# okieraised/rs-face-detection-tflite

Hardware: AMD Instinct MI355X
Metric: faces/sec at batch=256 (256x256 back-camera) per GPU (higher is better)
Workload: dtype f32

## Files before the change

rs-face-detection-tflite_amd/csrc/strip_kernels.hip:

```cpp
#include <hip/hip_runtime.h>

#include <algorithm>
#include <cstdint>
#include <cstdio>
#include <cstdlib>
#include <type_traits>

#include "kernels.hpp"
#include "launch.hpp"

namespace mi {

namespace {

typedef float sf32x16 __attribute__((ext_vector_type(16)));
typedef float v2f __attribute__((ext_vector_type(2)));
typedef float v4f __attribute__((ext_vector_type(4)));
typedef unsigned v2u __attribute__((ext_vector_type(2)));
typedef float __attribute__((address_space(4))) cfloat;

struct StripArgs {
    const float* in;
    float* out;
    const float* consts;
// ... 529 lines not shown
        if (has_skip) {
#pragma unroll
            for (int q = 0; q < CQ; q++) {
                oacc[2 * q] = v2f{mx[q].x, mx[q].y} + v2f{bp[4 * q], bp[4 * q + 1]};
                oacc[2 * q + 1] = v2f{mx[q].z, mx[q].w} + v2f{bp[4 * q + 2], bp[4 * q + 3]};
            }
        } else {
#pragma unroll
            for (int q = 0; q < CQ; q++) {
                oacc[2 * q] = v2f{bp[4 * q], bp[4 * q + 1]};
                oacc[2 * q + 1] = v2f{bp[4 * q + 2], bp[4 * q + 3]};
            }
        }
#pragma unroll
        for (int o = 0; o < 2 * CQ; o++) asm volatile("" : "+v"(oacc[o]));
    }
    load_first(0);
    load_x(0, xbuf[0]);
#pragma unroll
    for (int st = 0; st < 2 * CQ; st++) {
        const int q = st >> 1, h = st & 1;
        __builtin_amdgcn_s_waitcnt(0xC07F);
        if (MODE == 2) load_second(st);
        __builtin_amdgcn_sched_barrier(0);
        const float4 (&x)[3] = xbuf[q & 1];
        if (h == 0) {
            float4 m = make_float4(fmaxf(x[0].x, x[1].x), fmaxf(x[0].y, x[1].y), fmaxf(x[0].z, x[1].z), fmaxf(x[0].w, x[1].w));
            if (MODE == 0) m = make_float4(fmaxf(m.x, mx[q].x), fmaxf(m.y, mx[q].y), fmaxf(m.z, mx[q].z), fmaxf(m.w, mx[q].w));
            mx[q] = m;
        }
        v2f t[3];
#pragma unroll
        for (int kx = 0; kx < 3; kx++) t[kx] = h == 0 ? v2f{x[kx].x, x[kx].y} : v2f{x[kx].z, x[kx].w};
        auto wv = [&](int tap) { return v2f{wd[2 * tap], wd[2 * tap + 1]}; };
        v2f pch = acc[q][h], n;
        if (MODE == 0) {
            n = pch;
#pragma unroll
            for (int kx = 0; kx < 3; kx++) n = pkfma(t[kx], wv(3 + kx), n);
        } else {
            n = t[0] * wv(0);
#pragma unroll
            for (int kx = 0; kx < 3; kx++) {
                if (MODE == 2) pch = pkfma(t[kx], wv(6 + kx), pch);
                if (kx) n = pkfma(t[kx], wv(kx), n);
            }
        }
        acc[q][h] = n;
        asm volatile("" : "+v"(acc[q][h]));
        if constexpr (MODE == 2) {
#pragma unroll
            for (int o = 0; o < 2 * CQ; o++) oacc[o] = pkfma(v2f{pch.x, pch.x}, v2f{wp0[2 * o], wp0[2 * o + 1]}, oacc[o]);
            asm volatile("" : "+v"(pch));
        }
        __builtin_amdgcn_sched_barrier(0);
        __builtin_amdgcn_s_waitcnt(0xC07F);
        if (st + 1 < 2 * CQ) {
            load_first(st + 1);
            if (h == 1) load_x(q + 1, xbuf[(q + 1) & 1]);
        }
        __builtin_amdgcn_sched_barrier(0);
        if constexpr (MODE == 2) {
#pragma unroll
            for (int o = 0; o < 2 * CQ; o++) {
                oacc[o] = pkfma(v2f{pch.y, pch.y}, v2f{wp1[2 * o], wp1[2 * o + 1]}, oacc[o]);
                asm volatile("" : "+v"(oacc[o]));
            }
        }
        __builtin_amdgcn_sched_barrier(0);
    }
}

template <int CQ, int NH, int MODE, int PS>
__device__ __forceinline__ void strip_row_s2m(const float* me2, const cfloat* cst, int hf, bool has_skip, v2f (&acc)[CQ][2], float4 (&mx)[CQ],
                                              v4f (&oacc)[CQ], const float (&wa)[SK<CQ>::NA]) {
    constexpr int C = 4 * CQ, Co = NH * C;
    constexpr int ST2 = (32 + 2 * Co + 15) / 16 * 16, OFF_BIAS2 = (C / 2) * ST2;
    float wd[2][18];
    float4 xbuf[2][3];
    auto load_taps = [&](int st) {
        const cfloat* p = cst;
        asm volatile("" : "+s"(p));
#pragma unroll
        for (int i = 0; i < 18; i++) wd[st & 1][i] = p[st * ST2 + i];
    };
    auto load_x = [&](int q, float4 (&x)[3]) {
#pragma unroll
        for (int kx = 0; kx < 3; kx++) x[kx] = sld4(me2 + kx * PS + 4 * q);
    };
    if constexpr (MODE == 2) {
        const cfloat* bp = cst + OFF_BIAS2 + hf * C;
        asm volatile("" : "+s"(bp));
        if (has_skip) {
#pragma unroll
            for (int q = 0; q < CQ; q++) oacc[q] = v4f{mx[q].x, mx[q].y, mx[q].z, mx[q].w} + v4f{bp[4 * q], bp[4 * q + 1], bp[4 * q + 2], bp[4 * q + 3]};
        } else {
#pragma unroll
            for (int q = 0; q < CQ; q++) oacc[q] = v4f{bp[4 * q], bp[4 * q + 1], bp[4 * q + 2], bp[4 * q + 3]};
        }
#pragma unroll
        for (int q = 0; q < CQ; q++) asm volatile("" : "+v"(oacc[q]));
    }
    load_taps(0);
    load_x(0, xbuf[0]);
#pragma unroll
    for (int st = 0; st < 2 * CQ; st++) {
        const int q = st >> 1, h = st & 1;
        __builtin_amdgcn_s_waitcnt(0xC07F);
        if (st + 1 < 2 * CQ) {
            load_taps(st + 1);
            if (h == 1) load_x(q + 1, xbuf[(q + 1) & 1]);
        }
        __builtin_amdgcn_sched_barrier(0);
        const float4 (&x)[3] = xbuf[q & 1];
        if (h == 0) {
            float4 m = make_float4(fmaxf(x[0].x, x[1].x), fmaxf(x[0].y, x[1].y), fmaxf(x[0].z, x[1].z), fmaxf(x[0].w, x[1].w));
            if (MODE == 0) m = make_float4(fmaxf(m.x, mx[q].x), fmaxf(m.y, mx[q].y), fmaxf(m.z, mx[q].z), fmaxf(m.w, mx[q].w));
            mx[q] = m;
        }
        v2f t[3];
#pragma unroll
        for (int kx = 0; kx < 3; kx++) t[kx] = h == 0 ? v2f{x[kx].x, x[kx].y} : v2f{x[kx].z, x[kx].w};
        const float (&w)[18] = wd[st & 1];
        auto wv = [&](int tap) { return v2f{w[2 * tap], w[2 * tap + 1]}; };
        v2f pch = acc[q][h], n;
        if (MODE == 0) {
            n = pch;
#pragma unroll
            for (int kx = 0; kx < 3; kx++) n = pkfma(t[kx], wv(3 + kx), n);
        } else {
            n = t[0] * wv(0);
#pragma unroll
            for (int kx = 0; kx < 3; kx++) {
                if (MODE == 2) pch = pkfma(t[kx], wv(6 + kx), pch);
                if (kx) n = pkfma(t[kx], wv(kx), n);
            }
        }
        acc[q][h] = n;
        asm volatile("" : "+v"(acc[q][h]));
        if constexpr (MODE == 2) {
            asm volatile("" : "+v"(pch));
            __builtin_amdgcn_sched_barrier(0);
#pragma unroll
            for (int e = 0; e < 2; e++) {
                const float bv = e ? pch.y : pch.x;
#pragma unroll
                for (int tq = 0; tq < CQ; tq++) {
                    const int nn = (2 * st + e) * CQ + tq;
                    oacc[tq] = mfma4_bcast(wa[nn >> 4], bv, oacc[tq], nn & 15);
                }
            }
        }
        __builtin_amdgcn_sched_barrier(0);
    }
}

template <int CQ, bool RELU>
__global__ __launch_bounds__(256, CQ <= 6 ? 3 : 2) void strip_kernel(StripArgs a) {
    using K = SK<CQ>;
    constexpr int C = K::C, NL = K::NL, BUF_F = K::BUF_F;
    extern __shared__ __attribute__((aligned(16))) float lds[];
    const int lane = threadIdx.x & 63;
    const int wave = __builtin_amdgcn_readfirstlane(threadIdx.x >> 6);
    float* wbase = lds + wave * K::WAVE_F;
    int gw = blockIdx.x * 4 + wave;
    const int band = gw % a.bands;
    gw /= a.bands;
    const int strip = gw % a.strips, b = gw / a.strips;
    if (b >= a.B) return;
    const int x0 = strip * 64;
    const int y0 = band * a.band_rows, y1 = min(y0 + a.band_rows, a.H);
    if (y0 >= y1) return;
    const float* in = a.in + (long)b * a.in_fs;
    float* out = a.out + (long)b * a.out_fs;
    const cfloat* cst = (const cfloat*)a.consts;

    int goff[NL];
#pragma unroll
    for (int k = 0; k < NL; k++) {
        const int f = min(lane + 64 * k, K::NF - 1), px = f / CQ, qd = f - px * CQ;
        goff[k] = (min(max(x0 - 1 + px, 0), a.W - 1) * C + 4 * qd) * 4;
    }
    const int npx = min(64, a.W - x0);
    const bool full = npx == 64;
    const int zl = x0 == 0 ? 0 : -1;
    const int zr = x0 + 64 >= a.W ? npx + 1 : -1;
    const long gout = (long)x0 * C + 4 * lane;
    const unsigned lds_wave = __builtin_amdgcn_readfirstlane((unsigned)(uintptr_t)(__attribute__((address_space(3))) float*)wbase);

    auto issue_row = [&](int r, int bi) {
        const char* src = reinterpret_cast<const char*>(in + (long)min(max(r, 0), a.H - 1) * a.W * C);
        const unsigned dstb = lds_wave + (unsigned)(bi * BUF_F * 4);
        constexpr int TAIL = K::NF - 64 * (NL - 1);
#pragma unroll
        for (int k = 0; k < NL; k++) {
            if (k < NL - 1 || TAIL == 64) {
                asm volatile("s_mov_b32 m0, %0\n\ts_nop 0\n\tglobal_load_lds_dwordx4 %1, %2" ::"s"(dstb + 1024u * k), "v"(goff[k]), "s"(src) : "memory", "m0");
            } else {
                unsigned long long saved;
                asm volatile("s_mov_b64 %0, exec\n\ts_mov_b64 exec, %4\n\ts_mov_b32 m0, %1\n\ts_nop 0\n\tglobal_load_lds_dwordx4 %2, %3\n\ts_mov_b64 exec, %0"
                             : "=&s"(saved) : "s"(dstb + 1024u * k), "v"(goff[k]), "s"(src), "n"((1ull << (TAIL & 63)) - 1) : "memory", "m0");
            }
        }
    };
    const int zfix = lane < CQ ? (zl >= 0 ? zl * C + 4 * lane : -1) : (lane < 2 * CQ ? (zr >= 0 ? zr * C + 4 * (lane - CQ) : -1) : -1);
    auto fix_row = [&](int r, int bi) {
        float* buf = wbase + bi * BUF_F;
        const float4 z = make_float4(0.f, 0.f, 0.f, 0.f);
        if (r < 0 || r >= a.H) {
#pragma unroll
            for (int k = 0; k < NL; k++)
                if (64 * (k + 1) <= K::NF || lane < K::NF - 64 * k) sst4(buf + 4 * (lane + 64 * k), z);
        } else if (zfix >= 0) {
            sst4(buf + zfix, z);
        }
    };

    v2f oacc[2 * CQ];
    auto row = [&](auto emit_t, int bi, v2f (&aPN)[CQ][2], v2f (&aC)[CQ][2], const float4 (&xres)[CQ], float4 (&xcur)[CQ]) {
        strip_row<CQ, decltype(emit_t)::value>(wbase + bi * BUF_F + lane * C, cst, a.has_res != 0, aPN, aC, xres, xcur, oacc);
    };
    auto epilogue = [&](int y, int bi) {
        float* obuf = wbase + bi * BUF_F;
        float4 o[CQ];
        strip_act<CQ, RELU>(oacc, cst + K::OFF_SLOPE, a.hi, o);
#pragma unroll
        for (int q = 0; q < CQ; q++) sst4(obuf + lane * C + 4 * q, o[q]);
        wave_sync();
        float* dst = out + (long)y * a.W * C + gout;
        if (full) {
#pragma unroll
            for (int k = 0; k < CQ; k++) sst4(dst + 256 * k, sld4(obuf + 4 * lane + 256 * k));
        } else {
#pragma unroll
            for (int k = 0; k < CQ; k++) {
                const float4 o = sld4(obuf + 4 * lane + 256 * k);
                if (lane + 64 * k < npx * CQ) sst4(dst + 256 * k, o);
            }
        }
    };

    v2f acc0[CQ][2], acc1[CQ][2];
    float4 xa[CQ], xb[CQ];
#pragma unroll
    for (int q = 0; q < CQ; q++) {
        acc0[q][0] = acc0[q][1] = acc1[q][0] = acc1[q][1] = v2f{0.f, 0.f};
        xa[q] = xb[q] = make_float4(0.f, 0.f, 0.f, 0.f);
    }
#ifdef MI_STRIP_STAMPS
    unsigned long long st_acc[5] = {0, 0, 0, 0, 0}, st_prev = __builtin_amdgcn_s_memtime();
#define MI_SSTAMP(k) { __builtin_amdgcn_sched_barrier(0); unsigned long long t_ = __builtin_amdgcn_s_memtime(); __builtin_amdgcn_s_waitcnt(0xC07F); st_acc[k] += t_ - st_prev; st_prev = t_; __builtin_amdgcn_sched_barrier(0); }
#else
#define MI_SSTAMP(k)
#endif
    auto step = [&](auto emit, int r, v2f (&aPN)[CQ][2], v2f (&aC)[CQ][2], const float4 (&xprev)[CQ], float4 (&xcur)[CQ]) {
        const int bi = (r - (y0 - 1)) & 1;
        if (r + 1 <= y1) {
            if (full && r >= y0 + 2) wait_vm<NL + CQ>();
            else wait_vm<NL>();
        } else {
            wait_vm<0>();
        }
        MI_SSTAMP(0)
        fix_row(r, bi);
        wave_sync();
        MI_SSTAMP(1)
        row(emit, bi, aPN, aC, xprev, xcur);
        wave_sync();
        MI_SSTAMP(2)
        if constexpr (decltype(emit)::value) epilogue(r - 1, bi);
        wave_sync();
        if (r + 2 <= y1) issue_row(r + 2, bi);
        MI_SSTAMP(3)
    };
    issue_row(y0 - 1, 0);
    issue_row(y0, 1);
    step(std::false_type{}, y0 - 1, acc0, acc1, xb, xa);
    step(std::false_type{}, y0, acc1, acc0, xa, xb);
    for (int r = y0 + 1; r <= y1; r += 2) {
        step(std::true_type{}, r, acc0, acc1, xb, xa);
        if (r + 1 > y1) break;
        step(std::true_type{}, r + 1, acc1, acc0, xa, xb);
    }
#ifdef MI_STRIP_STAMPS
    if (a.stamps && lane == 0)
        for (int k = 0; k < 4; k++) a.stamps[((long)blockIdx.x * 4 + wave) * 8 + k] = st_acc[k];
#endif
}

constexpr int kMaxPipe = 4;
struct PipeArgs {
    const float* in;
    float* out;
    const float* consts[kMaxPipe];
    long in_fs, out_fs;
    int B, H, W;
    int strips, bands, band_rows, units;
    int rows_per_step;
    int has_res[kMaxPipe];
    float hi[kMaxPipe];
    int prio;
#ifdef MI_PIPE_STAMPS
    unsigned long long* stamps;
#endif
};

// ... 580 lines not shown
        const float4 z = make_float4(0.f, 0.f, 0.f, 0.f);
        if (e < 0 || e >= a.H) {
#pragma unroll
            for (int q = 0; q < CQ; q++) sst4(dstl + 4 * q, z);
        } else if (full) {
#pragma unroll
            for (int q = 0; q < CQ; q++) sst4(dstl + 4 * q, o[q]);
        } else {
#pragma unroll
            for (int q = 0; q < CQ; q++) sst4(dstl + 4 * q, lane >= npx ? z : o[q]);
        }
    };
    auto tail_step = [&](int t, v2f (&tacc)[CQ][2], float4 (&tmx)[CQ]) {
        if constexpr (NH2 > 0) {
            const int mt = t - 2 * S;
            if (mt < 0 || 2 * mt > a.band_rows) return;
            const int k = 2 * mt;
            constexpr int Co = NH2 * C;
            constexpr int ST2 = (32 + 2 * Co + 15) / 16 * 16, OFF_SLOPE2 = (C / 2) * ST2 + 64;
            const cfloat* cst2 = (const cfloat*)a.consts[S];
            const float* img = lds + ((S - 1) * 2) * IMG;
            const int tu = a.strips == 2 ? 0 : lane >> 5, tox = a.strips == 2 ? lane : lane & 31;
            const float* me2 = img + tu * 66 * C + (2 * tox + 1) * C;
            const bool skip = hf == 0 && a.has_res[S] != 0;
            if (mt == 0) {
                strip_row_s2<CQ, NH2, 1>(me2, cst2, hf, skip, tacc, tmx, oacc0);
            } else {
                strip_row_s2<CQ, NH2, 2>(me2, cst2, hf, skip, tacc, tmx, oacc0);
                float4 o[CQ];
                strip_act<CQ, RELU>(oacc0, cst2 + OFF_SLOPE2 + hf * C, a.hi[S], o);
                float* obuf = scratch;
#pragma unroll
                for (int q = 0; q < CQ; q++) sst4(obuf + lane * C + 4 * q, o[q]);
                wave_sync();
                const int Wo = a.W >> 1;
#pragma unroll
                for (int j = 0; j < CQ; j++) {
                    const int f = lane + 64 * j, px = f / CQ, qd = f - px * CQ;
                    const int u = a.strips == 2 ? 0 : px >> 5, ox = a.strips == 2 ? px : px & 31;
                    const int un = a.strips == 2 ? (int)blockIdx.x : 2 * (int)blockIdx.x + u;
                    const int ub = un % a.bands, bb = min(un / a.bands, a.B - 1);
                    const int uy0 = ub * a.band_rows, uy1 = min(uy0 + a.band_rows, a.H);
                    const float4 v = sld4(obuf + 4 * f);
                    if (un < a.units && uy0 + k <= uy1 && ox < Wo) {
                        const int oy = (uy0 + k - 2) >> 1;
                        sst4(a.out + (long)bb * a.out_fs + ((long)oy * Wo + ox) * Co + hf * C + 4 * qd, v);
                    }
                }
                wave_sync();
            }
            if (k + 1 < a.band_rows) strip_row_s2<CQ, NH2, 0>(me2 + IMG, cst2, hf, skip, tacc, tmx, oacc0);
        }
    };
    auto step = [&](int t, const float4 (&xin)[CQ], float4 (&xout)[CQ], v2f (&tacc)[CQ][2], float4 (&tmx)[CQ]) {
        const int m = t - 2 * role;
        const int c0 = lo_j - 1 + 2 * m;
        bool hand_over = false, store_out = false;
        float4 o0[CQ], o1[CQ];
        if (!tail && active && m >= 0 && m < P) {
            const float *me0, *me1;
            if (role == 0) {
                if (m + 1 < P) wait_vm<2 * NL>();
                else wait_vm<0>();
                fix_row(c0, (m & 1) * 2);
                fix_row(c0 + 1, (m & 1) * 2 + 1);
                wave_sync();
                me0 = scratch + ((m & 1) * 2) * BUF_F + lane * C;
                me1 = me0 + BUF_F;
            } else {
                me0 = lds + ((role - 1) * 2) * IMG + img_p + lane * C;
                me1 = me0 + IMG;
            }
            strip_row2<CQ>(me0, me1, cst, has_res, aA, aB, xin, xout, oacc0, oacc1);
            wave_sync();
            if (m >= 1) {
                strip_act<CQ, RELU>(oacc0, cst + K::OFF_SLOPE, hi, o0);
                strip_act<CQ, RELU>(oacc1, cst + K::OFF_SLOPE, hi, o1);
                if (NH2 || role < S - 1) hand_over = true;
#ifdef MI_ABL_STORE_EARLY
                else { store_row(c0 - 1, o0); store_row(c0, o1); }
#else
                else store_out = true;
#endif
            }
            if (role == 0 && m + 2 < P) {
                wave_sync();
                issue_row(c0 + 4, (m & 1) * 2);
                issue_row(c0 + 5, (m & 1) * 2 + 1);
            }
        }
        if constexpr (NH2 > 0) {
            if (tail) tail_step(t, tacc, tmx);
        }
        MI_PSTAMP(0)
        wg_barrier();
        MI_PSTAMP(1)
        if (hand_over) {
            hand_row(c0 - 1, 0, o0);
            hand_row(c0, 1, o1);
        } else if (store_out) {
            store_row(c0 - 1, o0);
            store_row(c0, o1);
        }
        MI_PSTAMP(2)
        wg_barrier();
        MI_PSTAMP(3)
    };
    const int T = NH2 ? 2 * S + a.band_rows / 2 + 1 : 2 * S - 1 + a.band_rows / 2;
    for (int t = 0; t < T; t += 2) {
        step(t, xa, xb, aA, xa);
        if (t + 1 >= T) break;
        step(t + 1, xb, xa, aA, xa);
    }
#ifdef MI_PIPE_STAMPS
    if (a.stamps && lane == 0) {
        unsigned long long* d = a.stamps + ((size_t)blockIdx.x * 8 + w) * 8;
        for (int k = 0; k < 4; k++) d[k] = ps_acc[k];
        d[4] = T;
    }
#endif
#undef MI_PSTAMP
}

template <int CQ, int KB, bool RELU, int NH2>
__global__ __launch_bounds__(NH2 ? 128 * (KB - 1) + 64 * NH2 : 128 * KB, 2) void strip_pipe2m_kernel(PipeArgs a) {
    using K = SK<CQ>;
    constexpr int C = K::C, NL = K::NL, BUF_F = K::BUF_F;
    constexpr int S = NH2 ? KB - 1 : KB;
    constexpr int NT = 128 * S + 64 * NH2;
    constexpr int PXS = C + 4;
    constexpr int IMG = 132 * PXS;
    constexpr int RING_F = (KB - 1) * 2 * IMG;
    extern __shared__ __attribute__((aligned(16))) float lds[];
    const int lane = threadIdx.x & 63;
    const int w = __builtin_amdgcn_readfirstlane(threadIdx.x >> 6);
    const bool tail = NH2 && w >= 2 * S;
    const int p = tail ? 0 : (w & 1), role = tail ? S : (w >> 1);
    const int hf = tail ? w - 2 * S : 0;
    {
        const bool first = role == 0, last = tail || (NH2 == 0 && role == S - 1);
        if ((a.prio == 1 && (first || last)) || (a.prio == 2 && first) || (a.prio == 3 && last)) __builtin_amdgcn_s_setprio(1);
    }
    float* scratch = lds + RING_F + (role == 0 ? p * 4 * BUF_F : 8 * BUF_F + (tail ? hf : p) * BUF_F);
    const int unit = a.strips == 2 ? (int)blockIdx.x : 2 * (int)blockIdx.x + p;
    const bool active = unit < a.units;
    const int band = unit % a.bands, b = min(unit / a.bands, a.B - 1);
    const int x0 = a.strips == 2 ? 64 * p : 0;
    const int y0 = band * a.band_rows, y1 = min(y0 + a.band_rows, a.H);
    const float* in = a.in + (long)b * a.in_fs;
    float* out = a.out + (long)b * a.out_fs;
    const cfloat* cst = (const cfloat*)a.consts[role];
    const bool has_res = a.has_res[role] != 0;
    const float hi = a.hi[role];
    const int hi_last = NH2 ? y1 + 2 : y1;
    const int lo_j = y0 - (S - 1 - role), hi_j = hi_last + (S - 1 - role);
    const int P = (hi_j - lo_j + 2) >> 1;
    const int img_p = a.strips == 2 ? 64 * PXS * p : 66 * PXS * p;

    for (int i = threadIdx.x; i < RING_F / 4; i += NT) reinterpret_cast<float4*>(lds)[i] = make_float4(0.f, 0.f, 0.f, 0.f);

    int goff[NL];
#pragma unroll
    for (int k = 0; k < NL; k++) {
        const int f = min(lane + 64 * k, K::NF - 1), px = f / CQ, qd = f - px * CQ;
        goff[k] = (min(max(x0 - 1 + px, 0), a.W - 1) * C + 4 * qd) * 4;
    }
    const int npx = min(64, a.W - x0);
    const bool full = npx == 64;
    const int zl = x0 == 0 ? 0 : -1;
    const int zr = x0 + 64 >= a.W ? npx + 1 : -1;
    const long gout = (long)x0 * C + 4 * lane;
    const unsigned lds_scratch = __builtin_amdgcn_readfirstlane((unsigned)(uintptr_t)(__attribute__((address_space(3))) float*)scratch);
    auto issue_row = [&](int r, int bi) {
        const char* src = reinterpret_cast<const char*>(in + (long)min(max(r, 0), a.H - 1) * a.W * C);
        const unsigned dstb = lds_scratch + (unsigned)(bi * BUF_F * 4);
        constexpr int TAIL = K::NF - 64 * (NL - 1);
#pragma unroll
        for (int k = 0; k < NL; k++) {
            if (k < NL - 1 || TAIL == 64) {
                asm volatile("s_mov_b32 m0, %0\n\ts_nop 0\n\tglobal_load_lds_dwordx4 %1, %2" ::"s"(dstb + 1024u * k), "v"(goff[k]), "s"(src) : "memory", "m0");
            } else {
                unsigned long long saved;
                asm volatile("s_mov_b64 %0, exec\n\ts_mov_b64 exec, %4\n\ts_mov_b32 m0, %1\n\ts_nop 0\n\tglobal_load_lds_dwordx4 %2, %3\n\ts_mov_b64 exec, %0"
                             : "=&s"(saved) : "s"(dstb + 1024u * k), "v"(goff[k]), "s"(src), "n"((1ull << (TAIL & 63)) - 1) : "memory", "m0");
            }
        }
    };
    const int zfix = lane < CQ ? (zl >= 0 ? zl * C + 4 * lane : -1) : (lane < 2 * CQ ? (zr >= 0 ? zr * C + 4 * (lane - CQ) : -1) : -1);
    auto fix_row = [&](int r, int bi) {
        float* buf = scratch + bi * BUF_F;
        const float4 z = make_float4(0.f, 0.f, 0.f, 0.f);
        if (r < 0 || r >= a.H) {
#pragma unroll
            for (int k = 0; k < NL; k++)
                if (64 * (k + 1) <= K::NF || lane < K::NF - 64 * k) sst4(buf + 4 * (lane + 64 * k), z);
        } else if (zfix >= 0) {
            sst4(buf + zfix, z);
        }
    };

    v2f aA[CQ][2], aB[CQ][2];
    v4f oacc0[CQ], oacc1[CQ];
    v4f toacc[CQ];
    float4 onext[CQ];
    float wa[K::NA];
    float cb[C], wd[2][18];
#pragma unroll
    for (int q = 0; q < CQ; q++) {
        aA[q][0] = aA[q][1] = aB[q][0] = aB[q][1] = v2f{0.f, 0.f};
        onext[q] = make_float4(0.f, 0.f, 0.f, 0.f);
    }
    auto prefetch_consts = [&]() {
        const cfloat* pc = cst;
        asm volatile("" : "+s"(pc));
#pragma unroll
        for (int i = 0; i < C; i++) cb[i] = pc[K::OFF_BIAS + i];
#pragma unroll
        for (int i = 0; i < 18; i++) wd[0][i] = pc[K::OFF_DW + i];
    };
    auto pin_consts = [&]() {
#pragma unroll
        for (int i = 0; i < C; i++) asm volatile("" : "+s"(cb[i]));
#pragma unroll
        for (int i = 0; i < 18; i++) asm volatile("" : "+s"(wd[0][i]));
    };
    if (!tail) {
#pragma unroll
        for (int i = 0; i < K::NA; i++) wa[i] = a.consts[role][K::OFF_A + 64 * i + lane];
    } else if constexpr (NH2 > 0) {
        constexpr int ST2h = (32 + 2 * NH2 * C + 15) / 16 * 16, OFF_A2 = (C / 2) * ST2h + 128;
#pragma unroll
        for (int i = 0; i < K::NA; i++) wa[i] = a.consts[S][OFF_A2 + (hf * K::NA + i) * 64 + lane];
    }
    prefetch_consts();
    if (role == 0 && active) {
        issue_row(lo_j - 1, 0);
        issue_row(lo_j, 1);
        if (P > 1) {
            issue_row(lo_j + 1, 2);
            issue_row(lo_j + 2, 3);
        }
    }
    __builtin_amdgcn_s_waitcnt(0xC07F);
    pin_consts();
    __builtin_amdgcn_s_barrier();
    if (!tail && !has_res) {
#pragma unroll
        for (int q = 0; q < CQ; q++) onext[q] = make_float4(cb[4 * q], cb[4 * q + 1], cb[4 * q + 2], cb[4 * q + 3]);
    }

#ifdef MI_PIPE_STAMPS
    unsigned long long ps_acc[7] = {0, 0, 0, 0, 0, 0, 0}, ps_prev = __builtin_amdgcn_s_memtime();
#define MI_PSTAMP(k) { __builtin_amdgcn_sched_barrier(0); unsigned long long t_ = __builtin_amdgcn_s_memtime(); __builtin_amdgcn_s_waitcnt(0xC07F); ps_acc[k] += t_ - ps_prev; ps_prev = t_; __builtin_amdgcn_sched_barrier(0); }
#else
#define MI_PSTAMP(k)
#endif
    auto wg_barrier = [&]() {
        asm volatile("" ::: "memory");
        __builtin_amdgcn_s_waitcnt(0xC07F);
#ifndef MI_ABL_NOBAR
        __builtin_amdgcn_s_barrier();
#endif
        asm volatile("" ::: "memory");
    };
    auto store_row = [&](int e, const float4 (&o)[CQ]) {
        float* obuf = scratch;
#pragma unroll
        for (int q = 0; q < CQ; q++) sst4(obuf + lane * C + 4 * q, o[q]);
        wave_sync();
        float* dst = out + (long)e * a.W * C + gout;
        if (full) {
#pragma unroll
            for (int k = 0; k < CQ; k++) sst4(dst + 256 * k, sld4(obuf + 4 * lane + 256 * k));
        } else {
#pragma unroll
            for (int k = 0; k < CQ; k++) {
                const float4 v = sld4(obuf + 4 * lane + 256 * k);
                if (lane + 64 * k < npx * CQ) sst4(dst + 256 * k, v);
            }
        }
        wave_sync();
    };
    auto hand_row = [&](int e, int which, const float4 (&o)[CQ]) {
        float* dstl = lds + (role * 2 + which) * IMG + img_p + (1 + lane) * PXS;
        const float4 z = make_float4(0.f, 0.f, 0.f, 0.f);
        if (e < 0 || e >= a.H) {
#pragma unroll
            for (int q = 0; q < CQ; q++) sst4(dstl + 4 * q, z);
        } else if (full) {
#pragma unroll
            for (int q = 0; q < CQ; q++) sst4(dstl + 4 * q, o[q]);
        } else {
#pragma unroll
            for (int q = 0; q < CQ; q++) sst4(dstl + 4 * q, lane >= npx ? z : o[q]);
        }
    };
    auto tail_step = [&](int t, v2f (&tacc)[CQ][2], float4 (&tmx)[CQ]) {
        if constexpr (NH2 > 0) {
            const int mt = t - 2 * S;
            if (mt < 0 || 2 * mt > a.band_rows) return;
            const int k = 2 * mt;
            constexpr int Co = NH2 * C;
            constexpr int ST2 = (32 + 2 * Co + 15) / 16 * 16, OFF_SLOPE2 = (C / 2) * ST2 + 64;
            const cfloat* cst2 = (const cfloat*)a.consts[S];
            const float* img = lds + ((S - 1) * 2) * IMG;
            const int tu = a.strips == 2 ? 0 : lane >> 5, tox = a.strips == 2 ? lane : lane & 31;
            const float* me2 = img + tu * 66 * PXS + (2 * tox + 1) * PXS;
            const bool skip = hf == 0 && a.has_res[S] != 0;
            if (mt == 0) {
                strip_row_s2m<CQ, NH2, 1, PXS>(me2, cst2, hf, skip, tacc, tmx, toacc, wa);
            } else {
                strip_row_s2m<CQ, NH2, 2, PXS>(me2, cst2, hf, skip, tacc, tmx, toacc, wa);
                float4 o[CQ];
                strip_act<CQ, RELU>(toacc, cst2 + OFF_SLOPE2 + hf * C, a.hi[S], o);
                float* obuf = scratch;
#pragma unroll
                for (int q = 0; q < CQ; q++) sst4(obuf + lane * C + 4 * q, o[q]);
                wave_sync();
                const int Wo = a.W >> 1;
#pragma unroll
                for (int j = 0; j < CQ; j++) {
                    const int f = lane + 64 * j, px = f / CQ, qd = f - px * CQ;
                    const int u = a.strips == 2 ? 0 : px >> 5, ox = a.strips == 2 ? px : px & 31;
                    const int un = a.strips == 2 ? (int)blockIdx.x : 2 * (int)blockIdx.x + u;
                    const int ub = un % a.bands, bb = min(un / a.bands, a.B - 1);
                    const int uy0 = ub * a.band_rows, uy1 = min(uy0 + a.band_rows, a.H);
                    const float4 v = sld4(obuf + 4 * f);
                    if (un < a.units && uy0 + k <= uy1 && ox < Wo) {
                        const int oy = (uy0 + k - 2) >> 1;
                        sst4(a.out + (long)bb * a.out_fs + ((long)oy * Wo + ox) * Co + hf * C + 4 * qd, v);
                    }
                }
                wave_sync();
            }
            if (k + 1 < a.band_rows) strip_row_s2m<CQ, NH2, 0, PXS>(me2 + IMG, cst2, hf, skip, tacc, tmx, toacc, wa);
        }
    };
    auto step = [&](int t) {
        v2f (&tacc)[CQ][2] = aA;
        float4 (&tmx)[CQ] = onext;
        const int m = t - 2 * role;
        const int c0 = lo_j - 1 + 2 * m;
        bool hand_over = false;
        float4 o0[CQ], o1[CQ];
        if (!tail && active && m >= 0 && m < P) {
            const float *me0, *me1;
            int ps;
            if (role == 0) {
                if (m + 1 < P) wait_vm<2 * NL>();
                else wait_vm<0>();
                fix_row(c0, (m & 1) * 2);
                fix_row(c0 + 1, (m & 1) * 2 + 1);
                wave_sync();
                me0 = scratch + ((m & 1) * 2) * BUF_F + lane * C;
                me1 = me0 + BUF_F;
                ps = C;
            } else {
                me0 = lds + ((role - 1) * 2) * IMG + img_p + lane * PXS;
                me1 = me0 + IMG;
                ps = PXS;
            }
            MI_PSTAMP(4)
            strip_row2m<CQ>(me0, me1, ps, cst, has_res, aA, aB, onext, oacc0, oacc1, wa, cb, wd);
            wave_sync();
            MI_PSTAMP(5)
            if (m >= 1) {
                strip_act<CQ, RELU>(oacc0, cst + K::OFF_SLOPE, hi, o0);
                strip_act<CQ, RELU>(oacc1, cst + K::OFF_SLOPE, hi, o1);
                if (NH2 || role < S - 1) hand_over = true;
                else { store_row(c0 - 1, o0); store_row(c0, o1); }
            }
            if (role == 0 && m + 2 < P) {
                wave_sync();
                issue_row(c0 + 4, (m & 1) * 2);
                issue_row(c0 + 5, (m & 1) * 2 + 1);
            }
        }
        if constexpr (NH2 > 0) {
            if (tail) tail_step(t, tacc, tmx);
        }
        MI_PSTAMP(6)
#ifdef MI_ABL_M_ONEBAR
        if (hand_over) {
            hand_row(c0 - 1, 0, o0);
            hand_row(c0, 1, o1);
        }
        MI_PSTAMP(1)
        MI_PSTAMP(2)
#else
        wg_barrier();
        MI_PSTAMP(1)
        if (hand_over) {
            hand_row(c0 - 1, 0, o0);
            hand_row(c0, 1, o1);
        }
        MI_PSTAMP(2)
#endif
        prefetch_consts();
        asm volatile("" ::: "memory");
        __builtin_amdgcn_s_waitcnt(0xC07F);
        pin_consts();
        __builtin_amdgcn_s_barrier();
        asm volatile("" ::: "memory");
        MI_PSTAMP(3)
    };
    const int T = NH2 ? 2 * S + a.band_rows / 2 + 1 : 2 * S - 1 + a.band_rows / 2;
    for (int t = 0; t < T; t++) step(t);
#ifdef MI_PIPE_STAMPS
    if (a.stamps && lane == 0) {
        unsigned long long* d = a.stamps + ((size_t)blockIdx.x * 8 + w) * 8;
        d[0] = ps_acc[4] + ps_acc[5] + ps_acc[6];
        for (int k = 1; k < 4; k++) d[k] = ps_acc[k];
        d[4] = T; d[5] = ps_acc[4]; d[6] = ps_acc[5]; d[7] = ps_acc[6];
    }
#endif
#undef MI_PSTAMP
}

template <int CQ, int KB, bool RELU, int NH2>
int launch_pipe_inst(const PipeArgs& pa, hipStream_t s) {
    using K = SK<CQ>;
    const bool two = pa.rows_per_step >= 2;
    if (pa.rows_per_step == 4) {
        auto k1 = strip_pipe1m_kernel<CQ, KB, RELU, NH2>;
        const size_t lds1 = (size_t)((KB - 1) * 2 * 132 * (K::C + 4) + 6 * K::BUF_F) * 4;
        if (hipError_t e = allow_full_lds(reinterpret_cast<const void*>(k1)); e != hipSuccess) return (int)e;
        const int wgs1 = pa.strips == 2 ? pa.units : (pa.units + 1) / 2;
        return (int)launch_kernel(k1, dim3((unsigned)wgs1), dim3(NH2 ? 128 * (KB - 1) + 64 * NH2 : 128 * KB), lds1, s, pa);
    }
    const bool mf = pa.rows_per_step == 3;
    auto kern = mf ? strip_pipe2m_kernel<CQ, KB, RELU, NH2> : (two ? strip_pipe2_kernel<CQ, KB, RELU, NH2> : strip_pipe_kernel<CQ, KB, RELU, NH2>);
    const size_t lds_bytes = (size_t)((KB - 1) * 2 * 132 * (mf ? K::C + 4 : K::C) + (two ? 10 : 6) * K::BUF_F) * 4;
    if (hipError_t e = allow_full_lds(reinterpret_cast<const void*>(kern)); e != hipSuccess) return (int)e;
    const int wgs = pa.strips == 2 ? pa.units : (pa.units + 1) / 2;
    return (int)launch_kernel(kern, dim3((unsigned)wgs), dim3(NH2 ? 128 * (KB - 1) + 64 * NH2 : 128 * KB), lds_bytes, s, pa);
}

unsigned long long* g_strip_stamps = nullptr;

int strips_band_rows(const BlockArgs& a, int strips) {
    static const int forced = getenv("MI_STRIP_BAND") ? atoi(getenv("MI_STRIP_BAND")) : 0;
    if (forced > 0) return std::min(forced, a.H);
    const long per_row_waves = (long)a.B * strips;
    long bands = std::max<long>(1, (3072 + per_row_waves / 2) / per_row_waves);
    int rows = (int)((a.H + bands - 1) / bands);
    const int floor_rows = per_row_waves * ((a.H + 11) / 12) >= 2048 ? 12
                         : (per_row_waves * ((a.H + 7) / 8) >= 1024 ? 8 : (per_row_waves * ((a.H + 3) / 4) >= 2048 ? 4 : (per_row_waves * ((a.H + 1) / 2) >= 2048 ? 2 : 1)));
    rows = std::max(rows, std::min(a.H, floor_rows));
    return rows;
}

template <int CQ, bool RELU>
int launch_strip_inst(const BlockArgs& a, hipStream_t s) {
    using K = SK<CQ>;
    auto kern = strip_kernel<CQ, RELU>;
    StripArgs sa;
    sa.in = a.in; sa.out = a.out; sa.consts = a.w_strip; sa.in_fs = a.in_fs; sa.out_fs = a.out_fs;
    sa.B = a.B; sa.H = a.H; sa.W = a.W;
    sa.strips = (a.W + 63) / 64;
    sa.band_rows = strips_band_rows(a, sa.strips);
    sa.bands = (a.H + sa.band_rows - 1) / sa.band_rows;
    sa.has_res = a.ep.res_mode == RES_DIRECT;
    sa.hi = a.ep.act == ACT_RELU6 ? 6.f : INFINITY;
    sa.stamps = g_strip_stamps;
    const long waves = (long)a.B * sa.strips * sa.bands;
    const size_t lds_bytes = (size_t)4 * K::WAVE_F * 4;
    if (hipError_t e = allow_full_lds(reinterpret_cast<const void*>(kern)); e != hipSuccess) return (int)e;
    return (int)launch_kernel(kern, dim3((unsigned)((waves + 3) / 4)), dim3(256), lds_bytes, s, sa);
}

}

bool strip_kernel_supports(const BlockArgs& a) {
    static const bool off = getenv("MI_NO_STRIP") != nullptr;
    if (off || !a.w_strip || !a.has_dw || a.sh != 1 || a.sw != 1 || a.pt != 1 || a.pl != 1) return false;
    if (a.C != a.Co || (a.C != 16 && a.C != 24 && a.C != 32) || a.H != a.Ho || a.W != a.Wo) return false;
    if (a.ep.res_mode != RES_NONE) {
        if (a.ep.res_after) return false;
        if (a.ep.res_mode != RES_DIRECT || a.ep.res != a.in || a.ep.res_fs != a.in_fs || a.ep.res_C != a.C) return false;
    }
    auto aligned16 = [](const void* p) { return (reinterpret_cast<uintptr_t>(p) & 15) == 0; };
    if (!aligned16(a.in) || !aligned16(a.out) || (a.in_fs & 3) || (a.out_fs & 3)) return false;
    return true;
}

bool strip_shape_ok(int C, int Co) { return C == Co && (C == 16 || C == 24 || C == 32); }

static int strip_stage_floats(int C) { return 32 + 2 * C + (16 - (2 * C) % 16) % 16; }
int strip_consts_floats(int C) { return C / 2 * strip_stage_floats(C) + 64 + 64 * ((C * (C / 4) + 15) / 16); }

void strip_pack_consts(int C, const float* w_dw, const float* b_dw, const float* w_pw, const float* bias, const float* alpha, int act, float* dst) {
    const int SF = strip_stage_floats(C);
    std::fill(dst, dst + strip_consts_floats(C), 0.f);
    for (int st = 0; st < C / 2; st++) {
        float* rec = dst + (size_t)st * SF;
        for (int t = 0; t < 9; t++)
            for (int e = 0; e < 2; e++) rec[2 * t + e] = w_dw[t * C + 2 * st + e];
        for (int half = 0; half < 2; half++)
            for (int o = 0; o < C; o++) rec[32 + half * C + o] = w_pw[(size_t)o * C + 2 * st + half];
    }
    float* pb = dst + (size_t)(C / 2) * SF;
    float* ps = pb + 32;
    for (int c = 0; c < C; c++) {
        double acc = bias ? bias[c] : 0.0;
        if (b_dw)
            for (int k = 0; k < C; k++) acc += (double)w_pw[(size_t)c * C + k] * b_dw[k];
        pb[c] = (float)acc;
        ps[c] = act == ACT_PRELU ? alpha[c] : (act == ACT_NONE ? 1.f : 0.f);
    }
    float* pa = ps + 32;
    const int CQ = C / 4;
    for (int k = 0; k < C; k++)
        for (int t = 0; t < CQ; t++)
            for (int i = 0; i < 4; i++) {
                const int n = k * CQ + t;
                pa[(n >> 4) * 64 + 4 * (n & 15) + i] = w_pw[(size_t)(4 * t + i) * C + k];
            }
}

const char* strip_kernel_label(const BlockArgs& a, char* buf, size_t cap) {
    snprintf(buf, cap, "strip_kernel<%d,%d>", a.C / 4, a.ep.act == ACT_RELU ? 1 : 0);
    return buf;
}

int launch_strip(const BlockArgs& a, void* stream) {
    hipStream_t s = (hipStream_t)stream;
    const bool relu = a.ep.act == ACT_RELU;
#define MI_STRIP_CASE(Q) \
    if (a.C == 4 * Q) return relu ? launch_strip_inst<Q, true>(a, s) : launch_strip_inst<Q, false>(a, s);
    MI_STRIP_CASE(4) MI_STRIP_CASE(6) MI_STRIP_CASE(8)
#undef MI_STRIP_CASE
    return (int)hipErrorInvalidValue;
}

static bool strip_tail_supports(const BlockArgs& t, const BlockArgs& first) {
    if (!t.w_strip || !t.has_dw || t.sh != 2 || t.sw != 2 || t.pt != 0 || t.pl != 0) return false;
    if (t.C != first.C || t.H != first.H || t.W != first.W || (t.H & 1) || (t.W & 1) || t.Ho * 2 != t.H || t.Wo * 2 != t.W) return false;
    if (t.Co != t.C && t.Co != 2 * t.C) return false;
    if (t.ep.res_mode != RES_NONE && (t.ep.res_mode != RES_MAXPOOL || t.ep.res_C != t.C || t.ep.res_H != t.H || t.ep.res_W != t.W)) return false;
    auto aligned16 = [](const void* p) { return (reinterpret_cast<uintptr_t>(p) & 15) == 0; };
    return aligned16(t.out) && !(t.out_fs & 3);
}

bool strip_pipe_supports(const BlockArgs* blocks, int n) {
    static const bool off = getenv("MI_NO_PIPE") != nullptr;
    if (off || n < 2 || n > kMaxPipe) return false;
    const bool tail = blocks[n - 1].sh == 2;
    for (int k = 0; k < n - (tail ? 1 : 0); k++) {
        BlockArgs t = blocks[k];
        if (k > 0) { t.in = blocks[0].in; t.in_fs = blocks[0].in_fs; if (t.ep.res_mode != RES_NONE) { t.ep.res = t.in; t.ep.res_fs = t.in_fs; } }
        if (k < n - 1) { t.out = blocks[0].in == blocks[n - 1].out ? t.out : const_cast<float*>(blocks[0].in); t.out_fs = blocks[0].in_fs; }
        if (!strip_kernel_supports(t)) return false;
        if (t.C != blocks[0].C || t.H != blocks[0].H || t.W != blocks[0].W) return false;
        if ((t.ep.act == ACT_RELU) != (blocks[0].ep.act == ACT_RELU)) return false;
    }
    if (tail) {
        if (!strip_tail_supports(blocks[n - 1], blocks[0])) return false;
        if ((blocks[n - 1].ep.act == ACT_RELU) != (blocks[0].ep.act == ACT_RELU)) return false;
        if (blocks[0].ep.act != ACT_RELU) return false;
// ... 110 lines not shown
```

Baseline: 220,800.

## Skip pipeline warm-up and tail steps when a strip covers the whole image

When there is a single band per image, the pipelined strip kernel now starts later (offset D) and skips the early steps that only process the zero-padded rows above the image. It also drops the extra trailing step, adding a flush routine that finishes the last stride-2 output row directly. Fewer pipeline steps means fewer workgroup barriers and less padding work per strip. Scratch buffer parity now follows the step index instead of the row index, which risks off-by-one errors in the row schedule.

Result: faster. 223,200, median of 6 (+1.1%).

```diff
diff --git a/rs-face-detection-tflite_amd/csrc/strip_kernels.hip b/rs-face-detection-tflite_amd/csrc/strip_kernels.hip
--- a/rs-face-detection-tflite_amd/csrc/strip_kernels.hip
+++ b/rs-face-detection-tflite_amd/csrc/strip_kernels.hip
@@ -705,6 +705,35 @@
             }
         }
         __builtin_amdgcn_sched_barrier(0);
+    }
+}
+
+template <int CQ, int NH>
+__device__ __forceinline__ void strip_flush_s2m(const cfloat* cst, int hf, bool has_skip, const v2f (&acc)[CQ][2], const float4 (&mx)[CQ],
+                                                v4f (&oacc)[CQ], const float (&wa)[SK<CQ>::NA]) {
+    constexpr int C = 4 * CQ, Co = NH * C;
+    constexpr int ST2 = (32 + 2 * Co + 15) / 16 * 16, OFF_BIAS2 = (C / 2) * ST2;
+    const cfloat* bp = cst + OFF_BIAS2 + hf * C;
+    asm volatile("" : "+s"(bp));
+    if (has_skip) {
+#pragma unroll
+        for (int q = 0; q < CQ; q++) oacc[q] = v4f{mx[q].x, mx[q].y, mx[q].z, mx[q].w} + v4f{bp[4 * q], bp[4 * q + 1], bp[4 * q + 2], bp[4 * q + 3]};
+    } else {
+#pragma unroll
+        for (int q = 0; q < CQ; q++) oacc[q] = v4f{bp[4 * q], bp[4 * q + 1], bp[4 * q + 2], bp[4 * q + 3]};
+    }
+#pragma unroll
+    for (int st = 0; st < 2 * CQ; st++) {
+        const v2f pch = acc[st >> 1][st & 1];
+#pragma unroll
+        for (int e = 0; e < 2; e++) {
+            const float bv = e ? pch.y : pch.x;
+#pragma unroll
+            for (int tq = 0; tq < CQ; tq++) {
+                const int nn = (2 * st + e) * CQ + tq;
+                oacc[tq] = mfma4_bcast(wa[nn >> 4], bv, oacc[tq], nn & 15);
+            }
+        }
     }
 }
 
@@ -1591,9 +1620,12 @@
     const cfloat* cst = (const cfloat*)a.consts[role];
     const bool has_res = a.has_res[role] != 0;
     const float hi = a.hi[role];
-    const int hi_last = NH2 ? y1 + 2 : y1;
+    const bool whole = a.bands == 1;
+    const int hi_last = NH2 && !whole ? y1 + 2 : y1;
     const int lo_j = y0 - (S - 1 - role), hi_j = hi_last + (S - 1 - role);
     const int P = (hi_j - lo_j + 2) >> 1;
+    const int D = whole ? S >> 1 : 0;
+    const int kskip = whole && !tail ? (S - role) >> 1 : 0;
     const int img_p = a.strips == 2 ? 64 * PXS * p : 66 * PXS * p;
 
     for (int i = threadIdx.x; i < RING_F / 4; i += NT) reinterpret_cast<float4*>(lds)[i] = make_float4(0.f, 0.f, 0.f, 0.f);
@@ -1673,11 +1705,12 @@
     }
     prefetch_consts();
     if (role == 0 && active) {
-        issue_row(lo_j - 1, 0);
-        issue_row(lo_j, 1);
-        if (P > 1) {
-            issue_row(lo_j + 1, 2);
-            issue_row(lo_j + 2, 3);
+        const int r0 = lo_j - 1 + 2 * D;
+        issue_row(r0, 0);
+        issue_row(r0 + 1, 1);
+        if (P - D > 1) {
+            issue_row(r0 + 2, 2);
+            issue_row(r0 + 3, 3);
         }
     }
     __builtin_amdgcn_s_waitcnt(0xC07F);
@@ -1736,7 +1769,7 @@
     };
     auto tail_step = [&](int t, v2f (&tacc)[CQ][2], float4 (&tmx)[CQ]) {
         if constexpr (NH2 > 0) {
-            const int mt = t - 2 * S;
+            const int mt = t + D - 2 * S;
             if (mt < 0 || 2 * mt > a.band_rows) return;
             const int k = 2 * mt;
             constexpr int Co = NH2 * C;
@@ -1746,10 +1779,7 @@
             const int tu = a.strips == 2 ? 0 : lane >> 5, tox = a.strips == 2 ? lane : lane & 31;
             const float* me2 = img + tu * 66 * PXS + (2 * tox + 1) * PXS;
             const bool skip = hf == 0 && a.has_res[S] != 0;
-            if (mt == 0) {
-                strip_row_s2m<CQ, NH2, 1, PXS>(me2, cst2, hf, skip, tacc, tmx, toacc, wa);
-            } else {
-                strip_row_s2m<CQ, NH2, 2, PXS>(me2, cst2, hf, skip, tacc, tmx, toacc, wa);
+            auto store_out = [&](int ke) {
                 float4 o[CQ];
                 strip_act<CQ, RELU>(toacc, cst2 + OFF_SLOPE2 + hf * C, a.hi[S], o);
                 float* obuf = scratch;
@@ -1765,33 +1795,44 @@
                     const int ub = un % a.bands, bb = min(un / a.bands, a.B - 1);
                     const int uy0 = ub * a.band_rows, uy1 = min(uy0 + a.band_rows, a.H);
                     const float4 v = sld4(obuf + 4 * f);
-                    if (un < a.units && uy0 + k <= uy1 && ox < Wo) {
-                        const int oy = (uy0 + k - 2) >> 1;
+                    if (un < a.units && uy0 + ke <= uy1 && ox < Wo) {
+                        const int oy = (uy0 + ke - 2) >> 1;
                         sst4(a.out + (long)bb * a.out_fs + ((long)oy * Wo + ox) * Co + hf * C + 4 * qd, v);
                     }
                 }
                 wave_sync();
+            };
+            if (mt == 0) {
+                strip_row_s2m<CQ, NH2, 1, PXS>(me2, cst2, hf, skip, tacc, tmx, toacc, wa);
+            } else {
+                strip_row_s2m<CQ, NH2, 2, PXS>(me2, cst2, hf, skip, tacc, tmx, toacc, wa);
+                store_out(k);
             }
             if (k + 1 < a.band_rows) strip_row_s2m<CQ, NH2, 0, PXS>(me2 + IMG, cst2, hf, skip, tacc, tmx, toacc, wa);
+            if (whole && k + 2 == a.band_rows) {
+                strip_flush_s2m<CQ, NH2>(cst2, hf, skip, tacc, tmx, toacc, wa);
+                store_out(k + 2);
+            }
         }
     };
     auto step = [&](int t) {
         v2f (&tacc)[CQ][2] = aA;
         float4 (&tmx)[CQ] = onext;
-        const int m = t - 2 * role;
+        const int m = t + D - 2 * role;
         const int c0 = lo_j - 1 + 2 * m;
+        const int bp = (t & 1) * 2;
         bool hand_over = false;
         float4 o0[CQ], o1[CQ];
-        if (!tail && active && m >= 0 && m < P) {
+        if (!tail && active && m >= kskip && m < P) {
             const float *me0, *me1;
             int ps;
             if (role == 0) {
                 if (m + 1 < P) wait_vm<2 * NL>();
                 else wait_vm<0>();
-                fix_row(c0, (m & 1) * 2);
-                fix_row(c0 + 1, (m & 1) * 2 + 1);
+                fix_row(c0, bp);
+                fix_row(c0 + 1, bp + 1);
                 wave_sync();
-                me0 = scratch + ((m & 1) * 2) * BUF_F + lane * C;
+                me0 = scratch + bp * BUF_F + lane * C;
                 me1 = me0 + BUF_F;
                 ps = C;
             } else {
@@ -1811,8 +1852,8 @@
             }
             if (role == 0 && m + 2 < P) {
                 wave_sync();
-                issue_row(c0 + 4, (m & 1) * 2);
-                issue_row(c0 + 5, (m & 1) * 2 + 1);
+                issue_row(c0 + 4, bp);
+                issue_row(c0 + 5, bp + 1);
             }
         }
         if constexpr (NH2 > 0) {
@@ -1843,7 +1884,7 @@
         asm volatile("" ::: "memory");
         MI_PSTAMP(3)
     };
-    const int T = NH2 ? 2 * S + a.band_rows / 2 + 1 : 2 * S - 1 + a.band_rows / 2;
+    const int T = (NH2 ? 2 * S + a.band_rows / 2 + (whole ? 0 : 1) : 2 * S - 1 + a.band_rows / 2) - D;
     for (int t = 0; t < T; t++) step(t);
 #ifdef MI_PIPE_STAMPS
     if (a.stamps && lane == 0) {
```
